# Traneptora/jxlatte

Hardware: AMD Instinct MI355X
Metric: Mpixels/s decoded (VarDCT 4K frame) at 1/2/4/8 MI355X vs host-CPU jxlatte (higher is better)
Workload: dtype f32; 1 GPU; vardct4k: 8 independent 3840x2160 VarDCT frames per GPU (mix=default, Gab + EPF x2 + XYB, f32 out), inputs resident in HBM; frames_per_gpu=8, frames_total=8, frame_seeds=1000 + i, frame i on rank i mod 1, distinct_frames=8, streams=2, kernel_launches_per_frame=2

## Files before the change

jxlatte_amd/csrc/epf_quot3.h:

```cpp
#pragma once
#include <hip/hip_runtime.h>

namespace jxl {

constexpr float kEpfQuotLo = 0x1p-100f;
constexpr float kEpfQuotHi = 0x1p+90f;

template <int NP>
__device__ __forceinline__ bool epf_quot3_in_window(const float n[3][NP]) {
    float lo = __builtin_fabsf(n[0][0]), sum = lo;
#pragma unroll
    for (int k = 1; k < 3 * NP; k++) {
        const float a = __builtin_fabsf(n[k % 3][k / 3]);
        lo = __builtin_fminf(lo, a);
        sum = sum + a;
    }
    return lo >= kEpfQuotLo && sum <= kEpfQuotHi;
}

__device__ __forceinline__ float epf_quot_refined_rcp(float d) {
    const float r0 = __builtin_amdgcn_rcpf(d);
    const float e0 = __builtin_fmaf(-d, r0, 1.0f);
    return __builtin_fmaf(e0, r0, r0);
}
__device__ __forceinline__ float epf_quot_by(float n, float d, float r1) {
    const float q0 = n * r1;
    const float e1 = __builtin_fmaf(-d, q0, n);
    const float q1 = __builtin_fmaf(e1, r1, q0);
    const float e2 = __builtin_fmaf(-d, q1, n);
    return __builtin_fmaf(e2, r1, q1);
}

template <int NP>
__device__ __forceinline__ void epf_quot3_patch(const float n[3][NP], const float d[NP], float out[3][NP]) {
    if (__builtin_expect(__builtin_amdgcn_ballot_w64(!epf_quot3_in_window<NP>(n)) == 0, 1)) {
#pragma unroll
        for (int i = 0; i < NP; i++) {
            const float r1 = epf_quot_refined_rcp(d[i]);
#pragma unroll
            for (int c = 0; c < 3; c++) out[c][i] = epf_quot_by(n[c][i], d[i], r1);
        }
    } else {
#pragma unroll
        for (int i = 0; i < NP; i++)
#pragma unroll
            for (int c = 0; c < 3; c++) out[c][i] = n[c][i] / d[i];
    }
}

__device__ __forceinline__ void epf_quot3(float n0, float n1, float n2, float d, float out[3]) {
    const float n[3][1] = {{n0}, {n1}, {n2}}, dd[1] = {d};
    float q[3][1];
    epf_quot3_patch<1>(n, dd, q);
    out[0] = q[0][0];
    out[1] = q[1][0];
    out[2] = q[2][0];
}

}
```

jxlatte_amd/csrc/restore_fused_body.h:

```cpp
#pragma once
#include <hip/hip_ext.h>
#include "jxl_internal.h"
#include <algorithm>
#include "restore_sink.h"
#include "epf_quot3.h"
#include <cstdlib>
#include <type_traits>

namespace jxl {

#ifndef JXL_EPF3_PH2_WAVES
#define JXL_EPF3_PH2_WAVES 2
#endif

namespace {

__device__ __forceinline__ int mirror_c(int c, int size) {
    while (c < 0 || c >= size) {
        const int tc = ~c;
        c = tc >= 0 ? tc : (size << 1) + tc;
    }
    return c;
}

template <bool GAB, int ITERS>
struct Geo {
    static constexpr int RG = GAB ? 1 : 0;
    static constexpr int R0 = (ITERS == 3 || ITERS == 4) ? 3 : 0;
    static constexpr int R1 = (ITERS >= 1 && ITERS <= 3) ? 2 : 0;
    static constexpr int R2 = (ITERS == 2 || ITERS == 3) ? 1 : 0;
    static constexpr int SHR = ITERS == 3 ? (R1 + R2) : ITERS == 2 ? R2 : 0;
#ifndef JXL_EPF0_WH
#define JXL_EPF0_WH 64
#endif
    static constexpr int WH = ITERS == 4 ? JXL_EPF0_WH : 32;
    static constexpr int OW = 64 - 2 * SHR, OH = WH - 2 * SHR;
    static constexpr int RE = R0 + R1 + R2;
    static constexpr int RT = RE + RG;
    static constexpr int IW = OW + 2 * RT, IH = OH + 2 * RT;
    static constexpr int SW = IW + 3;
    static constexpr int SH = IH + 1;
    static constexpr int PLANE = SW * SH;
    static constexpr size_t LDS_BYTES = sizeof(float) * (3 * PLANE + 16 * 16);
};

template <int PS>
__device__ __forceinline__ float adiff(const float* p, int u, int v, float s) {
    return u < v ? fabsf(p[u] - p[v]) * s : fabsf(p[v] - p[u]) * s;
}

template <int ITER, int SW, int PLANE, int PH, bool PLAINDIV = false, bool CHAINS = true>
__device__ __forceinline__ void epf_patch(const float* __restrict__ src, int ry, int rx, const float* s_inv ,
                                          const float* bmul , const EpfParams& ep, float res[3][4 * PH]) {
    constexpr int NP = 4 * PH;
    constexpr int R = ITER == 0 ? 3 : ITER == 1 ? 2 : 1;
    constexpr int NW = 4 + 2 * R, NH = PH + 2 * R;
    constexpr int NT = ITER == 0 ? 12 : 4;
    constexpr int TY[12] = {0, 0, -1, 1, -1, 1, 1, -1, 0, 0, 2, -2};
    constexpr int TX[12] = {-1, 1, 0, 0, 1, 1, -1, -1, -2, 2, 0, 0};
    constexpr int QY[5] = {0, 0, 0, -1, 1};
    constexpr int QX[5] = {0, -1, 1, 0, 0};

    float dist[NP][NT];
#pragma unroll
    for (int i = 0; i < NP; i++)
#pragma unroll
        for (int t = 0; t < NT; t++) dist[i][t] = 0.0f;

    if (ITER != 0 && CHAINS) {
        float hc[PH][5], vc[PH + 1][4];
        auto chain_channel = [&](int c, auto first_channel) {
            constexpr bool FIRST = decltype(first_channel)::value;
            float nb[NH * NW];
            const float* pc = src + c * PLANE + (ry - R) * SW + (rx - R);
#pragma unroll
            for (int y = 0; y < NH; y++)
#pragma unroll
                for (int x = 0; x < NW; x++) nb[y * NW + x] = pc[y * SW + x];
            const float sc = ep.channel_scale[c];
#pragma unroll
            for (int py = 0; py < PH; py++)
#pragma unroll
                for (int j = 0; j < 5; j++) {
                    const int cy = py + R, cx = j - 1 + R;
                    if (ITER == 2) {
                        const float t = adiff<NW>(nb, cy * NW + cx, cy * NW + cx + 1, sc);
                        hc[py][j] = FIRST ? t : hc[py][j] + t;
                    } else
#pragma unroll
                        for (int q = 0; q < 5; q++) {
                            const int u = (cy + QY[q]) * NW + cx + QX[q];
                            const float t = adiff<NW>(nb, u, u + 1, sc);
                            hc[py][j] = (FIRST && q == 0) ? t : hc[py][j] + t;
                        }
                }
            constexpr int I0 = 0;
#pragma unroll
            for (int i = I0; i <= PH; i++)
#pragma unroll
                for (int px = 0; px < 4; px++) {
                    const int cy = i - 1 + R, cx = px + R;
                    if (ITER == 2) {
                        const float t = adiff<NW>(nb, cy * NW + cx, (cy + 1) * NW + cx, sc);
                        vc[i][px] = FIRST ? t : vc[i][px] + t;
                    } else
#pragma unroll
                        for (int q = 0; q < 5; q++) {
                            const int u = (cy + QY[q]) * NW + cx + QX[q];
                            const float t = adiff<NW>(nb, u, u + NW, sc);
                            vc[i][px] = (FIRST && q == 0) ? t : vc[i][px] + t;
                        }
                }
        };
        chain_channel(0, std::true_type{});
#pragma unroll 1
        for (int c = 1; c < 3; c++) chain_channel(c, std::false_type{});
#pragma unroll
        for (int py = 0; py < PH; py++)
#pragma unroll
            for (int px = 0; px < 4; px++) {
                dist[py * 4 + px][0] = hc[py][px];
                dist[py * 4 + px][1] = hc[py][px + 1];
                dist[py * 4 + px][2] = vc[py][px];
                dist[py * 4 + px][3] = vc[py + 1][px];
            }
    } else {
    constexpr bool HROW = ITER == 0 && CHAINS && PH == 1;
    float h1[5], h2[6];
#pragma unroll
    for (int j = 0; j < 5; j++) h1[j] = 0.0f;
#pragma unroll
    for (int j = 0; j < 6; j++) h2[j] = 0.0f;
#pragma unroll 1
    for (int c = 0; c < 3; c++) {
        float nb[NH * NW];
        const float* pc = src + c * PLANE + (ry - R) * SW + (rx - R);
#pragma unroll
        for (int y = 0; y < NH; y++)
#pragma unroll
            for (int x = 0; x < NW; x++) nb[y * NW + x] = pc[y * SW + x];
        const float sc = ep.channel_scale[c];
#pragma unroll
        for (int py = 0; py < PH; py++)
#pragma unroll
            for (int px = 0; px < 4; px++) {
                const int cy = py + R, cx = px + R;
#pragma unroll
                for (int t = 0; t < NT; t++) {
                    if (HROW && TY[t] == 0) continue;
                    if (ITER == 2) {
                        dist[py * 4 + px][t] =
                            dist[py * 4 + px][t] + adiff<NW>(nb, cy * NW + cx, (cy + TY[t]) * NW + cx + TX[t], sc);
                    } else {
#pragma unroll
                        for (int q = 0; q < 5; q++) {
                            const int u = (cy + QY[q]) * NW + cx + QX[q];
                            const int v = (cy + TY[t] + QY[q]) * NW + cx + TX[t] + QX[q];
                            dist[py * 4 + px][t] = dist[py * 4 + px][t] + adiff<NW>(nb, u, v, sc);
                        }
                    }
                }
            }
        if (HROW) {
            constexpr int cy = R;
#pragma unroll
            for (int j = 0; j < 5; j++)
#pragma unroll
                for (int q = 0; q < 5; q++) {
                    const int u = (cy + QY[q]) * NW + (j - 1 + R) + QX[q];
                    h1[j] = h1[j] + adiff<NW>(nb, u, u + 1, sc);
                }
#pragma unroll
            for (int j = 0; j < 6; j++)
#pragma unroll
                for (int q = 0; q < 5; q++) {
                    const int u = (cy + QY[q]) * NW + (j - 2 + R) + QX[q];
                    h2[j] = h2[j] + adiff<NW>(nb, u, u + 2, sc);
                }
        }
    }
    if (HROW) {
#pragma unroll
        for (int px = 0; px < 4; px++)
#pragma unroll
            for (int t = 0; t < NT; t++) {
                if (TY[t] != 0) continue;
                dist[px][t] = TX[t] == -1 ? h1[px] : TX[t] == 1 ? h1[px + 1] : TX[t] == -2 ? h2[px] : h2[px + 2];
            }
    }
    }
    float sumW[NP];
    bool skip[NP];
#pragma unroll
    for (int i = 0; i < NP; i++) {
        const float s = s_inv[i];
        skip[i] = (s != s) || (s > (1.0f / 0.3f));
        float sw = 0.0f + 1.0f;
#pragma unroll
        for (int t = 0; t < NT; t++) {
            const float d = dist[i][t] * bmul[i];
            const float v = 1.0f - d * ep.sigma_scale * s;
            const float w = !PLAINDIV ? __builtin_fminf(__builtin_fmaxf(v, 0.0f), 1.0f) : __builtin_fmaxf(v, 0.0f);
            dist[i][t] = w;
            sw = sw + w;
        }
        sumW[i] = sw;
    }
    constexpr int RT2 = ITER == 0 ? 2 : 1;
    constexpr int MW = 4 + 2 * RT2, MH = PH + 2 * RT2;
    if constexpr (!PLAINDIV) {
        float num[3][NP];
#pragma unroll
        for (int c = 0; c < 3; c++) {
            float nb[MH * MW];
            const float* pc = src + c * PLANE + (ry - RT2) * SW + (rx - RT2);
#pragma unroll
            for (int y = 0; y < MH; y++)
#pragma unroll
                for (int x = 0; x < MW; x++) nb[y * MW + x] = pc[y * SW + x];
#pragma unroll
            for (int py = 0; py < PH; py++)
#pragma unroll
                for (int px = 0; px < 4; px++) {
                    const int i = py * 4 + px;
                    const int cy = py + RT2, cx = px + RT2;
                    float sc = 0.0f + nb[cy * MW + cx] * 1.0f;
#pragma unroll
                    for (int t = 0; t < NT; t++) sc = sc + nb[(cy + TY[t]) * MW + cx + TX[t]] * dist[i][t];
                    num[c][i] = sc;
                }
        }
        float q[3][NP];
        epf_quot3_patch<NP>(num, sumW, q);
#pragma unroll
        for (int py = 0; py < PH; py++)
#pragma unroll
            for (int px = 0; px < 4; px++)
#pragma unroll
                for (int c = 0; c < 3; c++) {
                    const int i = py * 4 + px;
                    float qv = q[c][i];
                    asm volatile("" : "+v"(qv));
                    res[c][i] = skip[i] ? src[c * PLANE + (ry + py) * SW + rx + px] : qv;
                }
        return;
    }
#pragma unroll
    for (int c = 0; c < 3; c++) {
        float nb[MH * MW];
        const float* pc = src + c * PLANE + (ry - RT2) * SW + (rx - RT2);
#pragma unroll
        for (int y = 0; y < MH; y++)
#pragma unroll
            for (int x = 0; x < MW; x++) nb[y * MW + x] = pc[y * SW + x];
#pragma unroll
        for (int py = 0; py < PH; py++)
#pragma unroll
            for (int px = 0; px < 4; px++) {
                const int i = py * 4 + px;
                const int cy = py + RT2, cx = px + RT2;
                float sc = 0.0f + nb[cy * MW + cx] * 1.0f;
#pragma unroll
                for (int t = 0; t < NT; t++) sc = sc + nb[(cy + TY[t]) * MW + cx + TX[t]] * dist[i][t];
#ifdef JXL_EPF_DIV_BRANCH
                res[c][i] = skip[i] ? nb[cy * MW + cx] : sc / sumW[i];
#else
                float qv = sc / sumW[i];
                asm volatile("" : "+v"(qv));
                res[c][i] = skip[i] ? nb[cy * MW + cx] : qv;
#endif
            }
    }
}

struct TileCtx {
    int ix0, iy0;
    int W, H;
    bool edge;
};

template <int PH, bool EDGE>
__device__ __forceinline__ void patch_sigma(int ry, int rx, const TileCtx& tc, const float* __restrict__ sig, int scy0, int scx0,
                                            const EpfParams& ep, float s_inv[4 * PH], float bmul[4 * PH]) {
    const int gx0 = tc.ix0 + rx;
    int cxa = (gx0 >> 3) - scx0, cxb = ((gx0 + 3) >> 3) - scx0;
    if (EDGE) {
        cxa = (min(max(gx0, 0), tc.W - 1) >> 3) - scx0;
        cxb = (min(max(gx0 + 3, 0), tc.W - 1) >> 3) - scx0;
    }
    const int first_n = 8 - (gx0 & 7);
    const uint32_t colb = 0x8181u >> (gx0 & 7);
#pragma unroll
    for (int py = 0; py < PH; py++) {
        const int gy = tc.iy0 + ry + py;
        const bool rowb = ((gy + 1) & 7) < 2;
        int crow = ((gy >> 3) - scy0) * 16;
        if (EDGE) crow = ((min(max(gy, 0), tc.H - 1) >> 3) - scy0) * 16;
        const float sa = sig[crow + cxa], sb = sig[crow + cxb];
        const uint32_t bm = rowb ? 0xfu : colb;
#pragma unroll
        for (int px = 0; px < 4; px++) {
            bmul[py * 4 + px] = (bm & (1u << px)) ? ep.border_sad_mul : 1.0f;
            s_inv[py * 4 + px] = px < first_n ? sa : sb;
        }
    }
}

template <int ITER, typename G, bool LAST, int PH, bool EDGE, bool PLAINDIV, typename Sink>
__device__ __forceinline__ void epf_stage(float* buf, int m, const TileCtx& tc, const float* __restrict__ sig, int scy0, int scx0,
                                          const EpfParams& ep, Sink sink) {
    constexpr int SW = G::SW, PLANE = G::PLANE;
    const int rw = G::IW - 2 * m, rh = G::IH - 2 * m;
    constexpr int NTHR = 512 / PH;
    const int pcols = (rw + 3) >> 2, prows = (rh + PH - 1) / PH;
    const int cblocks = (pcols + 7) >> 3, n_groups = cblocks * ((prows + 3) >> 2);
    const int q = threadIdx.x & 31;
    auto patch_of = [&](int g, int& prow, int& pcol) {
        pcol = (g % cblocks) * 8 + (q & 7);
        prow = (g / cblocks) * 4 + (q >> 3);
        return prow < prows && pcol < pcols;
    };
    if (LAST) {
        for (int g = threadIdx.x >> 5; g < n_groups; g += NTHR / 32) {
            int prow, pcol;
            if (!patch_of(g, prow, pcol)) continue;
            const int ry = m + prow * PH, rx = m + pcol * 4;
            float s_inv[4 * PH], bmul[4 * PH];
            patch_sigma<PH, EDGE>(ry, rx, tc, sig, scy0, scx0, ep, s_inv, bmul);
            float res[3][4 * PH];
            epf_patch<ITER, SW, PLANE, PH, PLAINDIV>(buf, ry, rx, s_inv, bmul, ep, res);
#pragma unroll
            for (int py = 0; py < PH; py++) {
                const int y = ry + py;
                if (y < G::IH - m) sink.row4(y, rx, &res[0][py * 4], &res[1][py * 4], &res[2][py * 4], min(4, G::IW - m - rx));
            }
        }
    } else {
        static_assert((64 / 4) * ((32 + PH - 1) / PH) <= NTHR, "one patch per thread");
        int prow, pcol;
        const bool act = patch_of(threadIdx.x >> 5, prow, pcol);
        const int ry = m + prow * PH, rx = m + pcol * 4;
        float res[3][4 * PH];
        if (act) {
            float s_inv[4 * PH], bmul[4 * PH];
            patch_sigma<PH, EDGE>(ry, rx, tc, sig, scy0, scx0, ep, s_inv, bmul);
            epf_patch<ITER, SW, PLANE, PH, PLAINDIV>(buf, ry, rx, s_inv, bmul, ep, res);
        }
        __syncthreads();
        if (act) {
#pragma unroll
            for (int py = 0; py < PH; py++) {
                const int y = ry + py;
#pragma unroll
                for (int px = 0; px < 4; px++) {
                    const int x = rx + px;
                    if (y < G::IH - m && x < G::IW - m) {
#pragma unroll
                        for (int c = 0; c < 3; c++) buf[c * PLANE + y * SW + x] = res[c][py * 4 + px];
                    }
                }
            }
        }
    }
}

template <typename G, int NTHR>
__device__ __forceinline__ void mirror_fixup(float* __restrict__ buf, int m, int rem, const TileCtx& tc) {
    const int rw = G::IW - 2 * m, rh = G::IH - 2 * m;
    __syncthreads();
    for (int i = threadIdx.x; i < rw * rh; i += NTHR) {
        const int y = m + i / rw, x = m + i % rw;
        const int gy = tc.iy0 + y, gx = tc.ix0 + x;
        const bool outside = gy < 0 || gy >= tc.H || gx < 0 || gx >= tc.W;
        const bool near = gy >= -rem && gy < tc.H + rem && gx >= -rem && gx < tc.W + rem;
        if (outside && near) {
            const int my = mirror_c(gy, tc.H) - tc.iy0, mx = mirror_c(gx, tc.W) - tc.ix0;
#pragma unroll
            for (int c = 0; c < 3; c++) buf[c * G::PLANE + y * G::SW + x] = buf[c * G::PLANE + my * G::SW + mx];
        }
    }
}


typedef float v2f_t __attribute__((ext_vector_type(2)));
struct __attribute__((packed, aligned(4))) f2a4 {
    float x, y;
};

template <int SK, bool NT = false, bool EDGE = true>
struct OutSink {
    const FusedArgs& a;
    const TileCtx& tc;
    __device__ __forceinline__ void colour(float& v0, float& v1, float& v2) const {
        if (a.p.xyb) invert_xyb_px(a.p.xybp, v0, v1, v2);
    }
    __device__ __forceinline__ void operator()(int y, int x, float v0, float v1, float v2) const {
        const int gy = tc.iy0 + y, gx = tc.ix0 + x;
        if (EDGE && (gy >= tc.H || gx >= tc.W)) return;
        colour(v0, v1, v2);
        sink_store_k<SK>(a, (uint32_t)(gy * tc.W + gx), v0, v1, v2);
    }
    __device__ __forceinline__ void row4(int y, int x, const float* r0, const float* r1, const float* r2, int nvalid) const {
        const int gy = tc.iy0 + y, gx = tc.ix0 + x;
        if (EDGE && gy >= tc.H) return;
        const int n = EDGE ? min(nvalid, tc.W - gx) : nvalid;
        if (n <= 0) return;
        float o[3][4];
#pragma unroll
        for (int i = 0; i < 4; i++) {
            o[0][i] = r0[i];
            o[1][i] = r1[i];
            o[2][i] = r2[i];
            colour(o[0][i], o[1][i], o[2][i]);
        }
        const uint32_t g = (uint32_t)(gy * tc.W + gx);
        if (n == 4 && (g & 1u) == 0 && sink_store4_k<SK, NT>(a, g, o)) return;
#pragma unroll
        for (int i = 0; i < 4; i++)
            if (i < n) sink_store_k<SK>(a, g + i, o[0][i], o[1][i], o[2][i]);
    }
};

template <bool GAB, int ITERS, int SK, int PH, bool EDGE, bool PLAINDIV>
__device__ __forceinline__ void restore_epf_stages(const FusedArgs& a, float* cur, int m, const TileCtx& tc, const float* __restrict__ sig,
                                                   int scy0, int scx0);

template <bool GAB, int ITERS, int SK, int PH, int LAY = 0, bool PLAINDIV = false>
__device__ __forceinline__ void restore_fused_body(const FusedArgs& a) {
    using G = Geo<GAB, ITERS>;
    constexpr int NTHR = 512 / PH;
    extern __shared__ float lds[];
    float* A = lds;
    float* sig = lds + 3 * G::PLANE;
    const int W = a.W, H = a.H;
    TileCtx tc;
    tc.W = W;
    tc.H = H;
    const int tiles_x = (W + G::OW - 1) / G::OW, tiles_y = (H + G::OH - 1) / G::OH;
    int ox, oy;
    {
        const int n_tiles = tiles_x * tiles_y;
        const int per_xcd = (n_tiles + 7) >> 3;
        const int tile = (int)(blockIdx.x & 7u) * per_xcd + (int)(blockIdx.x >> 3);
        if (tile >= n_tiles) return;
        ox = (tile % tiles_x) * G::OW;
        oy = (tile / tiles_x) * G::OH;
    }
    tc.ix0 = ox - G::RT;
    tc.iy0 = oy - G::RT;
    tc.edge = tc.ix0 < 0 || tc.iy0 < 0 || tc.ix0 + G::IW > W || tc.iy0 + G::IH > H;

    const int scy0 = max(tc.iy0, 0) >> 3, scx0 = max(tc.ix0, 0) >> 3;
    if (ITERS > 0 && threadIdx.x < 256) {
        const int cy = scy0 + (threadIdx.x >> 4), cx = scx0 + (threadIdx.x & 15);
        float v = 0.0f;
        if (cy < ((H + 7) >> 3) && cx < a.bw) v = a.inv_sigma[cy * a.bw + cx];
        sig[threadIdx.x] = v;
    }
    if (LAY == 1 && !tc.edge) {
        constexpr int NCX = (G::IW + 6) / 8 + 1, NCY = (G::IH + 6) / 8 + 1, TOTAL = NCX * NCY * 16;
        const int cells_w = W >> 3;
        const int ccy0 = tc.iy0 >> 3, ccx0 = tc.ix0 >> 3;
        const uint32_t base = (uint32_t)(ccy0 * cells_w + ccx0) << 6;
#pragma unroll
        for (int k = 0; k < (TOTAL + NTHR - 1) / NTHR; k++) {
            const int idx = (int)threadIdx.x + k * NTHR;
            const int cell = idx >> 4, pc = idx & 15;
            const int cyi = cell / NCX, cxi = cell - cyi * NCX;
            const int y = ((ccy0 + cyi) << 3) + (pc >> 1) - tc.iy0, x = ((ccx0 + cxi) << 3) + ((pc & 1) << 2) - tc.ix0;
            if ((TOTAL % NTHR == 0 || idx < TOTAL) && (unsigned)y < (unsigned)G::IH && x > -4 && x < G::IW) {
                const uint32_t g = base + ((uint32_t)(cyi * cells_w + cxi) << 6) + (uint32_t)(pc << 2);
                const float4 v0 = *reinterpret_cast<const float4*>(a.in[0] + g);
                const float4 v1 = *reinterpret_cast<const float4*>(a.in[1] + g);
                const float4 v2 = *reinterpret_cast<const float4*>(a.in[2] + g);
                float* d = A + y * G::SW + x;
                const float e0[4] = {v0.x, v0.y, v0.z, v0.w}, e1[4] = {v1.x, v1.y, v1.z, v1.w}, e2[4] = {v2.x, v2.y, v2.z, v2.w};
#pragma unroll
                for (int i = 0; i < 4; i++)
                    if ((unsigned)(x + i) < (unsigned)G::IW) {
                        d[i] = e0[i];
                        d[G::PLANE + i] = e1[i];
                        d[2 * G::PLANE + i] = e2[i];
                    }
            }
        }
    } else if (!tc.edge) {
        static_assert(G::IW % 2 == 0, "pairs");
        constexpr int PAIRS = G::IW / 2, TOTAL = PAIRS * G::IH;
        const uint32_t base = (uint32_t)(tc.iy0 * W + tc.ix0);
#pragma unroll
        for (int k = 0; k < (TOTAL + NTHR - 1) / NTHR; k++) {
            const int idx = (int)threadIdx.x + k * NTHR;
            if (idx < TOTAL) {
                const int y = idx / PAIRS, x = (idx - y * PAIRS) * 2;
                const uint32_t g = base + (uint32_t)(y * W + x);
                const f2a4 v0 = *reinterpret_cast<const f2a4*>(a.in[0] + g);
                const f2a4 v1 = *reinterpret_cast<const f2a4*>(a.in[1] + g);
                const f2a4 v2 = *reinterpret_cast<const f2a4*>(a.in[2] + g);
                float* d = A + y * G::SW + x;
                d[0] = v0.x;
                d[1] = v0.y;
                d[G::PLANE] = v1.x;
                d[G::PLANE + 1] = v1.y;
                d[2 * G::PLANE] = v2.x;
                d[2 * G::PLANE + 1] = v2.y;
            }
        }
    } else {
        constexpr int STEP_Y = NTHR / G::IW, STEP_X = NTHR % G::IW;
        int y = threadIdx.x / G::IW, x = threadIdx.x % G::IW;
        const float* __restrict__ in0 = a.in[0];
        const float* __restrict__ in1 = a.in[1];
        const float* __restrict__ in2 = a.in[2];
        while (y < G::IH) {
            int gy = tc.iy0 + y, gx = tc.ix0 + x;
            if (GAB) {
                gy = min(max(gy, 0), H - 1);
                gx = min(max(gx, 0), W - 1);
            } else {
                gy = mirror_c(gy, H);
                gx = mirror_c(gx, W);
            }
            const uint32_t g = LAY == 1 ? plane_tiled_off(W >> 3, gy, gx) : (uint32_t)(gy * W + gx);
            const float v0 = in0[g], v1 = in1[g], v2 = in2[g];
            float* d = A + y * G::SW + x;
            d[0] = v0;
            d[G::PLANE] = v1;
            d[2 * G::PLANE] = v2;
            x += STEP_X;
            y += STEP_Y;
            if (x >= G::IW) {
                x -= G::IW;
                y++;
            }
        }
    }
    __syncthreads();
    float* cur = A;
    int m = 0;
    if (GAB) {
        m = 1;
        constexpr int rw = G::IW - 2, rh = G::IH - 2;
        constexpr int NCOLSEG = NTHR / rw;
        constexpr int SEG = (rh + NCOLSEG - 1) / NCOLSEG;
        constexpr int NSEG = (rh + SEG - 1) / SEG;
        static_assert(NSEG * rw <= NTHR, "one pass");
        const int seg = threadIdx.x / rw, x = threadIdx.x - seg * rw;
        const int y0 = seg * SEG;
        float go[3][SEG];
        if (seg < NSEG) {
#pragma unroll
            for (int c = 0; c < 3; c++) {
                const float* p = cur + c * G::PLANE + y0 * G::SW + x;
                float a0 = p[0], a1 = p[1], a2 = p[2];
                float b0 = p[G::SW], b1 = p[G::SW + 1], b2 = p[G::SW + 2];
                float hs_a = a0 + a2;
                const float wb = a.p.gab_base[c], wa = a.p.gab_adj[c], wd = a.p.gab_diag[c];
#pragma unroll
                for (int k = 0; k < SEG; k++) {
                    if (y0 + k < rh) {
                        const float c0 = p[(k + 2) * G::SW], c1 = p[(k + 2) * G::SW + 1], c2 = p[(k + 2) * G::SW + 2];
                        const float hs_b = b0 + b2;
                        const float adj = hs_b + a1 + c1;
                        const float diag = hs_a + c0 + c2;
                        go[c][k] = wb * b1 + wa * adj + wd * diag;
                        a1 = b1;
                        hs_a = hs_b;
                        b0 = c0; b1 = c1; b2 = c2;
                    }
                }
            }
        }
        __syncthreads();
        if (seg < NSEG) {
#pragma unroll
            for (int c = 0; c < 3; c++) {
                float* o = cur + c * G::PLANE + (y0 + 1) * G::SW + x + 1;
#pragma unroll
                for (int k = 0; k < SEG; k++)
                    if (y0 + k < rh) o[k * G::SW] = go[c][k];
            }
        }
        if (tc.edge && ITERS > 0) mirror_fixup<G, NTHR>(cur, m, G::RE, tc);
        __syncthreads();
    }

    if (SK != SK_PLAIN || tc.edge) restore_epf_stages<GAB, ITERS, SK, PH, true, PLAINDIV>(a, cur, m, tc, sig, scy0, scx0);
    else restore_epf_stages<GAB, ITERS, SK, PH, false, PLAINDIV>(a, cur, m, tc, sig, scy0, scx0);
}

template <bool GAB, int ITERS, int SK, int PH, bool EDGE, bool PLAINDIV>
__device__ __forceinline__ void restore_epf_stages(const FusedArgs& a, float* cur, int m, const TileCtx& tc, const float* __restrict__ sig,
                                                   int scy0, int scx0) {
    using G = Geo<GAB, ITERS>;
    constexpr int NTHR = 512 / PH;
    const OutSink<SK, (ITERS != 4), EDGE> sink{a, tc};

    if (ITERS == 0) {
        const int mm = m;
        for (int i = threadIdx.x; i < G::OW * G::OH; i += NTHR) {
            const int y = mm + i / G::OW, x = mm + i % G::OW;
            sink(y, x, cur[y * G::SW + x], cur[G::PLANE + y * G::SW + x], cur[2 * G::PLANE + y * G::SW + x]);
        }
        return;
    }
    if (ITERS == 4) {
        m += 3;
        epf_stage<0, G, true, PH, EDGE, PLAINDIV>(cur, m, tc, sig, scy0, scx0, a.p.epf[0], sink);
        return;
    }
    if (ITERS == 3) {
        m += 3;
        epf_stage<0, G, false, PH, EDGE, PLAINDIV>(cur, m, tc, sig, scy0, scx0, a.p.epf[0], sink);
        if (EDGE) mirror_fixup<G, NTHR>(cur, m, G::R1 + G::R2, tc);
        __syncthreads();
    }
    m += 2;
    if (ITERS >= 2) {
        epf_stage<1, G, false, PH, EDGE, PLAINDIV>(cur, m, tc, sig, scy0, scx0, a.p.epf[1], sink);
        if (EDGE) mirror_fixup<G, NTHR>(cur, m, G::R2, tc);
        __syncthreads();
        m += 1;
        epf_stage<2, G, true, PH, EDGE, PLAINDIV>(cur, m, tc, sig, scy0, scx0, a.p.epf[2], sink);
    } else {
        epf_stage<1, G, true, PH, EDGE, PLAINDIV>(cur, m, tc, sig, scy0, scx0, a.p.epf[1], sink);
    }
}

#define JXL_RESTORE_BOUNDS(ITERS, PH) __launch_bounds__(512 / PH, ITERS >= 3 ? (PH == 1 ? 4 : JXL_EPF3_PH2_WAVES) : PH == 1 ? 8 : 4)
template <bool GAB, int ITERS, int SK, int PH, int LAY = 0, bool PLAINDIV = false>
__global__ JXL_RESTORE_BOUNDS(ITERS, PH) void k_restore_fused(const FusedArgs a) {
    restore_fused_body<GAB, ITERS, SK, PH, LAY, PLAINDIV>(a);
}

template <bool GAB, int ITERS, int SK, bool PLAINDIV = false>
__global__ JXL_RESTORE_BOUNDS(ITERS, 1) void k_restore_fused_batch(const FusedArgs* __restrict__ args) {
    typedef const __attribute__((address_space(4))) FusedArgs* cargs;
    restore_fused_body<GAB, ITERS, SK, 1, 0, PLAINDIV>(*(const FusedArgs*)((cargs)args + blockIdx.y));
}

template <bool GAB, int ITERS, int SK, int PH, int LAY = 0, bool PLAINDIV = false>
void launch_tph(const FusedArgs& a, hipStream_t s) {
    using G = Geo<GAB, ITERS>;
    if constexpr (ITERS > 0 && !PLAINDIV) {
        if (epf_weights_plain(a.p)) return launch_tph<GAB, ITERS, SK, PH, LAY, true>(a, s);
    }
    static const size_t pad = getenv("JXL_RESTORE_LDS_PAD") ? (size_t)atoi(getenv("JXL_RESTORE_LDS_PAD")) : 0;
    static bool attr_set = false;
    if (!attr_set) {
        (void)hipFuncSetAttribute(reinterpret_cast<const void*>(&k_restore_fused<GAB, ITERS, SK, PH, LAY, PLAINDIV>),
                                  hipFuncAttributeMaxDynamicSharedMemorySize, (int)(G::LDS_BYTES + pad));
        attr_set = true;
    }
    const int tiles_x = (a.W + G::OW - 1) / G::OW, tiles_y = (a.H + G::OH - 1) / G::OH;
    const int n_tiles = tiles_x * tiles_y;
    const dim3 grid(((n_tiles + 7) / 8) * 8);
    if (g_restore_kernel_ev[0] && g_restore_kernel_ev[1])
        hipExtLaunchKernelGGL((k_restore_fused<GAB, ITERS, SK, PH, LAY, PLAINDIV>), grid, dim3(512 / PH), (uint32_t)(G::LDS_BYTES + pad), s, g_restore_kernel_ev[0],
                              g_restore_kernel_ev[1], 0u, a);
    else
        hipLaunchKernelGGL((k_restore_fused<GAB, ITERS, SK, PH, LAY, PLAINDIV>), grid, dim3(512 / PH), G::LDS_BYTES + pad, s, a);
}

template <bool GAB, int ITERS, int SK, bool PLAINDIV = false>
void launch_batch_t(const FusedArgs* host_args, const FusedArgs* dev_args, int n, hipStream_t s) {
    using G = Geo<GAB, ITERS>;
    if constexpr (ITERS > 0 && !PLAINDIV) {
        if (epf_weights_plain(host_args[0].p)) return launch_batch_t<GAB, ITERS, SK, true>(host_args, dev_args, n, s);
    }
    static bool attr_set = false;
    if (!attr_set) {
        (void)hipFuncSetAttribute(reinterpret_cast<const void*>(&k_restore_fused_batch<GAB, ITERS, SK, PLAINDIV>),
                                  hipFuncAttributeMaxDynamicSharedMemorySize, (int)G::LDS_BYTES);
        attr_set = true;
    }
    int max_tiles = 0;
    for (int i = 0; i < n; i++)
        max_tiles = std::max(max_tiles, ((host_args[i].W + G::OW - 1) / G::OW) * ((host_args[i].H + G::OH - 1) / G::OH));
    const dim3 grid(((max_tiles + 7) / 8) * 8, n);
    hipLaunchKernelGGL((k_restore_fused_batch<GAB, ITERS, SK, PLAINDIV>), grid, dim3(512), G::LDS_BYTES, s, dev_args);
}

template <int SK>
void launch_fused_sk(const FusedArgs& a, hipStream_t s) {
    const int it = a.p.epf_iters;
    if (a.tiled) {
        if (a.p.gab) {
            if (it == 0) launch_tph<true, 0, SK, 1, 1>(a, s);
            else if (it == 1) launch_tph<true, 1, SK, 1, 1>(a, s);
            else launch_tph<true, 2, SK, 1, 1>(a, s);
        } else {
            if (it == 0) launch_tph<false, 0, SK, 1, 1>(a, s);
            else if (it == 1) launch_tph<false, 1, SK, 1, 1>(a, s);
            else launch_tph<false, 2, SK, 1, 1>(a, s);
        }
        return;
    }
    if (a.p.gab) {
        if (it == 0) launch_tph<true, 0, SK, 1>(a, s);
        else if (it == 1) launch_tph<true, 1, SK, 1>(a, s);
        else if (it == 2) launch_tph<true, 2, SK, 1>(a, s);
        else if (it == 4) {
            if constexpr (SK == SK_PLAIN) launch_tph<true, 4, SK_PLAIN, 1>(a, s);
        } else launch_tph<true, 3, SK, 1>(a, s);
    } else {
        if (it == 0) launch_tph<false, 0, SK, 1>(a, s);
        else if (it == 1) launch_tph<false, 1, SK, 1>(a, s);
        else if (it == 2) launch_tph<false, 2, SK, 1>(a, s);
        else if (it == 4) {
            if constexpr (SK == SK_PLAIN) launch_tph<false, 4, SK_PLAIN, 1>(a, s);
        } else launch_tph<false, 3, SK, 1>(a, s);
    }
}
template <int SK>
void launch_fused_batch_sk(const FusedArgs* h, const FusedArgs* d, int n, hipStream_t s) {
    const int it = h[0].p.epf_iters;
    if (h[0].p.gab) {
        if (it == 0) launch_batch_t<true, 0, SK>(h, d, n, s);
        else if (it == 1) launch_batch_t<true, 1, SK>(h, d, n, s);
        else if (it == 2) launch_batch_t<true, 2, SK>(h, d, n, s);
        else launch_batch_t<true, 3, SK>(h, d, n, s);
    } else {
        if (it == 0) launch_batch_t<false, 0, SK>(h, d, n, s);
        else if (it == 1) launch_batch_t<false, 1, SK>(h, d, n, s);
        else if (it == 2) launch_batch_t<false, 2, SK>(h, d, n, s);
        else launch_batch_t<false, 3, SK>(h, d, n, s);
    }
}

}
}
```

Before: 62900 Mpixels/s.

## Strength-reduce LAY1 tile load, pad LDS front, fold skip test into sigma

The cell-layout tile load now computes lane coordinates once and advances them incrementally instead of recomputing division and modulo per iteration. LDS gets a 3-float front pad so partial-edge float4 pieces can be written unconditionally without per-element bounds checks. The skip decision is folded into the staged inverse sigma (set to infinity when NaN or above threshold) and applied inside the quotient patch callback, which removes a separate select loop. The risks are that writes landing in the front pad or past the row could clobber neighbouring LDS data, and that the dropped idx<TOTAL guard could let out-of-range lanes do extra loads.

```diff
diff --git a/jxlatte_amd/csrc/epf_quot3.h b/jxlatte_amd/csrc/epf_quot3.h
--- a/jxlatte_amd/csrc/epf_quot3.h
+++ b/jxlatte_amd/csrc/epf_quot3.h
@@ -31,8 +31,8 @@
     return __builtin_fmaf(e2, r1, q1);
 }
 
-template <int NP>
-__device__ __forceinline__ void epf_quot3_patch(const float n[3][NP], const float d[NP], float out[3][NP]) {
+template <int NP, typename Plain>
+__device__ __forceinline__ void epf_quot3_patch(const float n[3][NP], const float d[NP], float out[3][NP], Plain plain) {
     if (__builtin_expect(__builtin_amdgcn_ballot_w64(!epf_quot3_in_window<NP>(n)) == 0, 1)) {
 #pragma unroll
         for (int i = 0; i < NP; i++) {
@@ -44,8 +44,12 @@
 #pragma unroll
         for (int i = 0; i < NP; i++)
 #pragma unroll
-            for (int c = 0; c < 3; c++) out[c][i] = n[c][i] / d[i];
+            for (int c = 0; c < 3; c++) out[c][i] = plain(c, i, n[c][i] / d[i]);
     }
+}
+template <int NP>
+__device__ __forceinline__ void epf_quot3_patch(const float n[3][NP], const float d[NP], float out[3][NP]) {
+    epf_quot3_patch<NP>(n, d, out, [](int, int, float q) { return q; });
 }
 
 __device__ __forceinline__ void epf_quot3(float n0, float n1, float n2, float d, float out[3]) {
diff --git a/jxlatte_amd/csrc/restore_fused_body.h b/jxlatte_amd/csrc/restore_fused_body.h
--- a/jxlatte_amd/csrc/restore_fused_body.h
+++ b/jxlatte_amd/csrc/restore_fused_body.h
@@ -230,19 +230,10 @@
                     num[c][i] = sc;
                 }
         }
-        float q[3][NP];
-        epf_quot3_patch<NP>(num, sumW, q);
-#pragma unroll
-        for (int py = 0; py < PH; py++)
-#pragma unroll
-            for (int px = 0; px < 4; px++)
-#pragma unroll
-                for (int c = 0; c < 3; c++) {
-                    const int i = py * 4 + px;
-                    float qv = q[c][i];
-                    asm volatile("" : "+v"(qv));
-                    res[c][i] = skip[i] ? src[c * PLANE + (ry + py) * SW + rx + px] : qv;
-                }
+        epf_quot3_patch<NP>(num, sumW, res, [&](int c, int i, float q) {
+            const float s = s_inv[i];
+            return ((s != s) || (s > (1.0f / 0.3f))) ? src[c * PLANE + (ry + i / 4) * SW + rx + i % 4] : q;
+        });
         return;
     }
 #pragma unroll
@@ -430,7 +421,8 @@
     using G = Geo<GAB, ITERS>;
     constexpr int NTHR = 512 / PH;
     extern __shared__ float lds[];
-    float* A = lds;
+    constexpr int FRONT = LAY == 1 ? 3 : 0;
+    float* A = lds + FRONT;
     float* sig = lds + 3 * G::PLANE;
     const int W = a.W, H = a.H;
     TileCtx tc;
@@ -455,33 +447,45 @@
         const int cy = scy0 + (threadIdx.x >> 4), cx = scx0 + (threadIdx.x & 15);
         float v = 0.0f;
         if (cy < ((H + 7) >> 3) && cx < a.bw) v = a.inv_sigma[cy * a.bw + cx];
+        if (v != v || v > (1.0f / 0.3f)) v = __builtin_inff();
         sig[threadIdx.x] = v;
     }
     if (LAY == 1 && !tc.edge) {
         constexpr int NCX = (G::IW + 6) / 8 + 1, NCY = (G::IH + 6) / 8 + 1, TOTAL = NCX * NCY * 16;
         const int cells_w = W >> 3;
         const int ccy0 = tc.iy0 >> 3, ccx0 = tc.ix0 >> 3;
-        const uint32_t base = (uint32_t)(ccy0 * cells_w + ccx0) << 6;
+        static_assert(NTHR % 16 == 0, "a lane keeps its piece index");
+        constexpr int CSTEP = NTHR / 16, DY = CSTEP / NCX, DX = CSTEP % NCX;
+        const int pc = threadIdx.x & 15;
+        const int cyi0 = (int)(threadIdx.x >> 4) / NCX;
+        int cxi = (int)(threadIdx.x >> 4) - cyi0 * NCX;
+        int y = ((ccy0 + cyi0) << 3) + (pc >> 1) - tc.iy0, x = ((ccx0 + cxi) << 3) + ((pc & 1) << 2) - tc.ix0;
+        const size_t tile0 = (size_t)(uint32_t)(ccy0 * cells_w + ccx0) << 6;
+        const char* const in0 = reinterpret_cast<const char*>(a.in[0] + tile0);
+        const char* const in1 = reinterpret_cast<const char*>(a.in[1] + tile0);
+        const char* const in2 = reinterpret_cast<const char*>(a.in[2] + tile0);
+        uint32_t g = ((uint32_t)(cyi0 * cells_w + cxi) << 8) + (uint32_t)(pc << 4);
+        const uint32_t gstep = (uint32_t)(DY * cells_w + DX) << 8, gwrap = (uint32_t)(cells_w - NCX) << 8;
 #pragma unroll
         for (int k = 0; k < (TOTAL + NTHR - 1) / NTHR; k++) {
-            const int idx = (int)threadIdx.x + k * NTHR;
-            const int cell = idx >> 4, pc = idx & 15;
-            const int cyi = cell / NCX, cxi = cell - cyi * NCX;
-            const int y = ((ccy0 + cyi) << 3) + (pc >> 1) - tc.iy0, x = ((ccx0 + cxi) << 3) + ((pc & 1) << 2) - tc.ix0;
-            if ((TOTAL % NTHR == 0 || idx < TOTAL) && (unsigned)y < (unsigned)G::IH && x > -4 && x < G::IW) {
-                const uint32_t g = base + ((uint32_t)(cyi * cells_w + cxi) << 6) + (uint32_t)(pc << 2);
-                const float4 v0 = *reinterpret_cast<const float4*>(a.in[0] + g);
-                const float4 v1 = *reinterpret_cast<const float4*>(a.in[1] + g);
-                const float4 v2 = *reinterpret_cast<const float4*>(a.in[2] + g);
+            if ((unsigned)y < (unsigned)G::IH && (unsigned)(x + 3) < (unsigned)(G::IW + 3)) {
+                const float4 v0 = *reinterpret_cast<const float4*>(in0 + g);
+                const float4 v1 = *reinterpret_cast<const float4*>(in1 + g);
+                const float4 v2 = *reinterpret_cast<const float4*>(in2 + g);
                 float* d = A + y * G::SW + x;
-                const float e0[4] = {v0.x, v0.y, v0.z, v0.w}, e1[4] = {v1.x, v1.y, v1.z, v1.w}, e2[4] = {v2.x, v2.y, v2.z, v2.w};
-#pragma unroll
-                for (int i = 0; i < 4; i++)
-                    if ((unsigned)(x + i) < (unsigned)G::IW) {
-                        d[i] = e0[i];
-                        d[G::PLANE + i] = e1[i];
-                        d[2 * G::PLANE + i] = e2[i];
-                    }
+                d[0] = v0.x, d[1] = v0.y, d[2] = v0.z, d[3] = v0.w;
+                d[G::PLANE] = v1.x, d[G::PLANE + 1] = v1.y, d[G::PLANE + 2] = v1.z, d[G::PLANE + 3] = v1.w;
+                d[2 * G::PLANE] = v2.x, d[2 * G::PLANE + 1] = v2.y, d[2 * G::PLANE + 2] = v2.z, d[2 * G::PLANE + 3] = v2.w;
+            }
+            cxi += DX;
+            y += 8 * DY;
+            x += 8 * DX;
+            g += gstep;
+            if (cxi >= NCX) {
+                cxi -= NCX;
+                y += 8;
+                x -= 8 * NCX;
+                g += gwrap;
             }
         }
     } else if (!tc.edge) {
```

Result: faster. 64350 Mpixels/s, median of 6 (+2.3%).
